# hannesweisbach/channelcoding

Hardware: AMD Instinct MI355X
Metric: decoded frames/sec (coded bits/sec = value x 255), BCH(255,231) min-sum, batch=2^20 (higher is better)
Workload: dtype f32

## Files before the change

channelcoding_amd/csrc/cc_internal.hpp:

```cpp
#pragma once
#include <hip/hip_runtime.h>

#include <cstdint>
#include <memory>
#include <mutex>
#include <string>
#include <vector>

#include "../../include/channelcoding_amd.h"
#include "galois.hpp"

namespace ccamd {

struct MinSumGeometry {
  int W = 64, C = 4, frames_per_wave = 1, KW = 1;
};

struct MinSumParams {
  int n, K, KW;
  int variant;
  int stop_rule;
  unsigned iterations;
  float alpha_f;
  float beta_f;
// ... 158 lines not shown
                           const uint32_t *d_er_off, uint8_t *d_out, int32_t *d_nerr, int32_t *d_status, size_t B,
                           hipStream_t stream, int il = 1);
int launch_chase(const cc_code *code, const float *d_llr, unsigned p, uint8_t *d_out, int32_t *d_nerr, float *d_metric,
                 int32_t *d_status, size_t B, hipStream_t stream);
int chase_frames_per_wave(const cc_code *code, unsigned p, bool soft, bool extended = false);
int launch_chase_soft(const cc_code *code, const float *d_llr, unsigned p, float beta, uint8_t *d_out, float *d_ext,
                      int32_t *d_nerr, float *d_metric, int32_t *d_status, size_t B, hipStream_t stream);
int launch_chase_extended(const cc_code *code, const float *d_llr, unsigned p, float beta, uint8_t *d_out, float *d_ext,
                          int32_t *d_nerr, float *d_metric, int32_t *d_status, size_t B, hipStream_t stream);
int launch_osd(const cc_code *code, const float *d_llr, unsigned order, uint8_t *d_out, int32_t *d_nerr, float *d_metric,
               int32_t *d_status, size_t B, hipStream_t stream);
int osd_frames_per_wave(const cc_code *code);
std::vector<unsigned long long> build_osd_rows(const CodeTables &t);
int launch_gmd(const cc_code *code, const uint8_t *d_words, const float *d_rel, unsigned m, uint8_t *d_out, int32_t *d_nerr,
               float *d_metric, int32_t *d_status, size_t B, hipStream_t stream);
bool bitslice_supported(const cc_code *code);
int launch_bitslice_syndromes(const cc_code *code, bool float_in, const void *d_in, uint8_t *d_out, uint8_t *d_synd, size_t B,
                              hipStream_t stream, int il = 1);
bool bitslice_encode_supported(const cc_code *code);
int launch_bitslice_encode(const cc_code *code, const uint8_t *d_msg, uint8_t *d_cw, size_t B, hipStream_t stream, int il = 1);
int launch_bitslice_chien(const void *d_lamp, void *d_masks, size_t B, bool long_locators, hipStream_t stream);
int launch_bitslice_roots_transpose(const void *d_masks, void *d_rootsT, size_t B, hipStream_t stream);
constexpr uint32_t kLogZero = 512;
int launch_chunk_bm(const cc_code *code, const uint8_t *d_synd, const uint16_t *d_er, const uint32_t *d_er_off,
                    uint16_t *d_llg, uint16_t *d_meta, unsigned long long *d_mask, uint8_t *d_lamp, int ncoef,
                    uint32_t *d_nleft, int32_t *d_nerr, int32_t *d_status, size_t B, hipStream_t stream);
int algebraic_route(const cc_code *code, size_t B, bool erasures);
bool planes_small_call(const cc_code *code, size_t B);
int launch_pgz_erasures(const cc_code *code, const uint8_t *d_in, const uint16_t *d_er, const uint32_t *d_er_off,
                        uint8_t *d_out, int32_t *d_nerr, int32_t *d_status, size_t B, hipStream_t stream);
constexpr int diag_variant_part(int variant, int parts) {
  const int order = variant == CC_ALG_MS ? 0 : variant == CC_ALG_NMS ? 1 : variant == CC_ALG_OMS ? 2
                  : variant == CC_ALG_SCMS2 ? 3 : variant == CC_ALG_SCMS1 ? 4 : 5;
  return order % parts;
}

enum DiagRowBody { DIAG_ROWS_BUTTERFLY = 0, DIAG_ROWS_FOUR = 1, DIAG_ROWS_FOUR_PIPELINED = 2, DIAG_ROWS_FOUR_ZIPPED = 3 };
constexpr int diag_row_body(int K, int D, int LPF, int variant) {
  const bool plain = variant == CC_ALG_MS || variant == CC_ALG_NMS || variant == CC_ALG_OMS || variant == CC_ALG_2DNMS;
  if (!(K == 24 && D == 7 && LPF == 16 && plain)) return DIAG_ROWS_BUTTERFLY;
#ifdef CC_DIAG_FOUR_ROW_BODY
  return CC_DIAG_FOUR_ROW_BODY;
#else
  return DIAG_ROWS_FOUR_ZIPPED;
#endif
}

constexpr bool diag_switch_from_registers(int K, int D, int LPF, int variant) {
  if (LPF != 8) return true;
  if (K == 28 && D == 7) return false;
  if (variant == CC_ALG_SCMS2) return !((K == 21 && D == 6) || (K == 10 && D == 1) || (K == 8 && D == 1));
  if (variant == CC_ALG_SCMS1) return !((K == 20 && D == 1) || (K == 24 && D == 4));
  return true;
}

int launch_wide_correct(const cc_code *code, const uint16_t *d_in, const uint16_t *d_er, const uint32_t *d_off,
                        uint16_t *d_out, int32_t *d_nerr, int32_t *d_status, size_t B, hipStream_t stream);
int launch_wide_pgz_erasures(const cc_code *code, const uint16_t *d_in, const uint16_t *d_er, const uint32_t *d_off,
                        uint16_t *d_out, int32_t *d_nerr, int32_t *d_status, size_t B, hipStream_t stream);
int launch_wide_encode(const cc_code *code, const uint16_t *d_msg, uint16_t *d_cw, size_t B, hipStream_t stream);
int launch_wide_extract(const cc_code *code, const uint16_t *d_cw, uint16_t *d_msg, size_t B, hipStream_t stream);
std::vector<uint8_t> build_parity_table(const Field &f, const CodeTables &t);
int launch_encode(const cc_code *code, const uint8_t *d_msg, uint8_t *d_cw, size_t B, hipStream_t stream);
int launch_encode_bits(const cc_code *code, const uint8_t *d_msg, uint8_t *d_cw, size_t B, hipStream_t stream);
int launch_extract(const cc_code *code, const uint8_t *d_cw, uint8_t *d_msg, size_t B, hipStream_t stream);
int launch_pack_bits(const void *d_sym, int width, size_t n, uint8_t *d_packed, size_t B, hipStream_t stream);
int launch_unpack_bits(const uint8_t *d_packed, size_t n, void *d_sym, int width, size_t B, hipStream_t stream);
bool packed_native_supported(const cc_code *code, size_t B);
int launch_packed_correct(const cc_code *code, const uint8_t *d_in, uint8_t *d_out, int32_t *d_nerr, int32_t *d_status,
                          size_t B, hipStream_t stream);
bool packed_long_supported(const cc_code *code, size_t B);
int launch_packed_long_correct(const cc_code *code, const uint8_t *d_in, uint8_t *d_out, int32_t *d_nerr, int32_t *d_status,
                               size_t B, hipStream_t stream);
bool packed_encode_native(const cc_code *code);
bool packed_extract_native(const cc_code *code);
int launch_packed_encode(const cc_code *code, const uint8_t *d_msg, uint8_t *d_cw, size_t B, hipStream_t stream);
int launch_packed_extract(const cc_code *code, const uint8_t *d_cw, uint8_t *d_msg, size_t B, hipStream_t stream);
constexpr size_t kInterleaveMax = 256;
constexpr size_t kInterleaveNativeMax = 16;
int launch_interleave(const void *d_in, int width, size_t n, size_t I, void *d_out, size_t B, bool to_interleaved,
                      hipStream_t stream);
bool interleaved_native_supported(const cc_code *code, size_t B, size_t I, bool erasures);
bool interleaved_encode_native(const cc_code *code, size_t I);
bool interleaved_extract_native(const cc_code *code, size_t I);
int launch_interleaved_extract(const cc_code *code, const void *d_cw, void *d_msg, size_t B, size_t I, hipStream_t stream);
struct ProductShape {
  int e;
  size_t w1, w2, k1, k2, N;
};
ProductShape product_shape(const cc_product *pc);
size_t product_chunk_blocks(size_t N, size_t blocks, size_t at_least = 1);
int launch_product_decode(const cc_product *pc, const float *d_y, uint8_t *d_out, float *d_ext, int32_t *d_status, size_t B,
                          hipStream_t stream);
int launch_product_encode(const cc_product *pc, const uint8_t *d_msg, uint8_t *d_cw, size_t B, hipStream_t stream);
int launch_product_extract(const cc_product *pc, const uint8_t *d_cw, uint8_t *d_msg, size_t B, hipStream_t stream);
int product_awgn(const cc_product *pc, double ebno_db, uint64_t seed, uint64_t first_block, size_t blocks,
                 int random_codewords, float *d_y, uint8_t *d_sent, hipStream_t stream);
int mc_run_product(const cc_product *pc, double ebno_db, uint64_t seed, uint64_t first_block, size_t blocks,
                   int random_codewords, uint64_t *d_counters, hipStream_t stream);
int mc_run_product_hard(const cc_product *pc, double ebno_db, uint64_t seed, uint64_t first_block, size_t blocks,
                        int random_codewords, uint64_t *d_counters, hipStream_t stream);
int launch_product_hard(const cc_product *pc, const uint8_t *d_in, uint8_t *d_out, int32_t *d_nflip, int32_t *d_last,
                        int32_t *d_status, size_t B, hipStream_t stream);
struct SrSchedule {
  int D = 0;
  float u[CC_PRODUCT_SR_MAX_LEVELS] = {};
// ... 74 lines not shown
```

channelcoding_amd/csrc/minsum_diag.hip:

```cpp
#include "minsum_diag_impl.hpp"

#include <algorithm>
#include <cstdlib>

namespace ccamd {

using DiagLaunch = int (*)(const cc_code *, const MinSumParams &, const float *, const uint16_t *, const uint32_t *,
                           uint8_t *, float *, uint16_t *, int32_t *, size_t, hipStream_t);
#define CC_PART_DECL(NAME, I)                                                                                        \
  int launch_minsum_diag_##NAME##_p##I(const cc_code *, const MinSumParams &, const float *, const uint16_t *,       \
                                       const uint32_t *, uint8_t *, float *, uint16_t *, int32_t *, size_t, hipStream_t);
#define CC_PARTS_1(M, NAME) M(NAME, 0)
#define CC_PARTS_2(M, NAME) CC_PARTS_1(M, NAME) M(NAME, 1)
#define CC_PARTS_3(M, NAME) CC_PARTS_2(M, NAME) M(NAME, 2)
#define CC_PARTS_6(M, NAME) CC_PARTS_3(M, NAME) M(NAME, 3) M(NAME, 4) M(NAME, 5)
#define GEO(NAME, N, KK, W, DD, LL, CC, OO, SC, PA, LK, PP) CC_PARTS_##PP(CC_PART_DECL, NAME)
#include "minsum_diag_geos.inc"
#undef GEO
namespace {
struct DiagEntry {
  DiagGeometry geo;
  int parts;
  DiagLaunch launch[6];
};
// ... 150 lines not shown
    return mx * 1000 + sq;
  };
  bool improved = true;
  while (improved) {
    improved = false;
    for (int a = 0; a < D && !improved; ++a)
      for (int b = a + 1; b < D && !improved; ++b)
        for (size_t x = 0; x < grp[a].size() && !improved; ++x)
          for (size_t y = 0; y < grp[b].size() && !improved; ++y) {
            const int before = group_cost(grp[a]) + group_cost(grp[b]);
            std::swap(grp[a][x], grp[b][y]);
            if (group_cost(grp[a]) + group_cost(grp[b]) < before)
              improved = true;
            else
              std::swap(grp[a][x], grp[b][y]);
          }
  }
  std::vector<uint16_t> out(static_cast<size_t>(D) * W, 0xFFFFu);
  for (int g = 0; g < D; ++g)
    for (size_t l = 0; l < grp[g].size(); ++l) out[g * W + l] = static_cast<uint16_t>(grp[g][l]);
  (void)real_last;
  return out;
}

bool minsum_diag_supported(const cc_code *code) {
  if (code->d_diag == nullptr || code->desc.iterations == 0) return false;
  const int alg = code->desc.algorithm;
  const DiagGeometry *geo = diag_geometry(code->tab);
  if (!geo) return false;
  if (alg == CC_ALG_SCMS1) return true;
  if (alg == CC_ALG_SCMS2) return geo->scms;
  if (alg != CC_ALG_MS && alg != CC_ALG_NMS && alg != CC_ALG_OMS && alg != CC_ALG_2DNMS) return false;
  if (alg == CC_ALG_OMS && !(code->desc.beta >= 0.0)) return false;
  const float a = static_cast<float>(code->desc.alpha);
  if ((alg == CC_ALG_NMS || alg == CC_ALG_2DNMS) && !(a == a && a - a == 0.0f)) return false;
  return diag_geometry(code->tab) != nullptr;
}


std::string minsum_diag_name(const cc_code *code) {
  const DiagGeometry *g = diag_geometry(code->tab);
  if (!g) return "minsum_diag_kernel";
  const int body = diag_row_body(static_cast<int>(g->k), g->D, g->LPF, code->desc.algorithm);
  return "minsum_diag_kernel<K=" + std::to_string(g->k) + ",D=" + std::to_string(g->D) + ",LPF=" + std::to_string(g->LPF) +
         (body == DIAG_ROWS_FOUR_ZIPPED      ? ",four-row-zipped>"
          : body == DIAG_ROWS_FOUR_PIPELINED ? ",four-row-pipelined>"
          : body == DIAG_ROWS_FOUR           ? ",four-row>"
                                             : ",row-pipelined>");
}

size_t minsum_diag_lds_bytes(const DiagGeometry &g) {
  const bool partial = g.w != static_cast<unsigned>(g.LPF * g.D);
  const size_t fpw = 64 / g.LPF, rc = static_cast<size_t>(g.LPF) * g.CPL + (partial ? 48 : (g.LPF == 8 && g.CPL == 8 ? 8 : 16));
  return 4 * (fpw * rc * 8 + (fpw / 2) * rc * 8) + 256 * 4 +
         4 * static_cast<size_t>(g.CPL) * 256;
}


namespace {

__global__ void __launch_bounds__(256)
twopass_gather_kernel(const uint32_t *__restrict__ ctl, unsigned sample, unsigned cap, const uint32_t *__restrict__ list,
                      const float *__restrict__ llr, float *__restrict__ llr2, int n) {
  if (!two_pass_in_effect(ctl, sample, cap)) return;
  const unsigned long long cnt = ctl[1];
  const int lane = threadIdx.x & 63;
  const unsigned long long nwaves = static_cast<unsigned long long>(gridDim.x) * 4;
  for (unsigned long long k = static_cast<unsigned long long>(blockIdx.x) * 4 + (threadIdx.x >> 6); k < cnt; k += nwaves) {
    const float *src = llr + static_cast<unsigned long long>(list[k]) * n;
    float *dst = llr2 + k * n;
    for (int j = lane; j < n; j += 64) dst[j] = src[j];
  }
}
__global__ void __launch_bounds__(256)
twopass_scatter_kernel(const uint32_t *__restrict__ ctl, unsigned sample, unsigned cap, const uint32_t *__restrict__ list,
                       const uint8_t *__restrict__ hard2, const uint16_t *__restrict__ iters2,
                       const int32_t *__restrict__ status2, uint8_t *__restrict__ hard, uint16_t *__restrict__ iters,
                       int32_t *__restrict__ status, int n) {
  if (!two_pass_in_effect(ctl, sample, cap)) return;
  const unsigned long long cnt = ctl[1];
  const int lane = threadIdx.x & 63;
  const unsigned long long nwaves = static_cast<unsigned long long>(gridDim.x) * 4;
  for (unsigned long long k = static_cast<unsigned long long>(blockIdx.x) * 4 + (threadIdx.x >> 6); k < cnt; k += nwaves) {
    const unsigned long long f = list[k];
    for (int j = lane; j < n; j += 64) hard[f * n + j] = hard2[k * n + j];
    if (lane == 0) {
      if (iters) iters[f] = iters2[k];
      if (status) status[f] = status2[k];
    }
  }
}

bool two_pass_enabled() { return minsum_shortcuts_enabled(); }

int launch_two_pass(const cc_code *code, const DiagEntry *e, const MinSumParams &p, const float *d_llr, uint8_t *d_hard,
                    uint16_t *d_iters, int32_t *d_status, size_t B, hipStream_t stream) {
  const size_t n = code->tab.n, cap = B / 4, sample = 4096;
  auto up = [](size_t v) { return (v + 255) & ~static_cast<size_t>(255); };
  constexpr size_t max_runs = 4, o_pool = 256, pool_bytes = POOL_WORDS * 4;
  const size_t o_list = o_pool + (max_runs + 2) * pool_bytes, o_llr = o_list + up(cap * 4), o_hard = o_llr + up(cap * n * 4),
               o_it = o_hard + up(cap * n), o_st = o_it + up(cap * 2), total = o_st + up(cap * 4);
  uint8_t *ws = nullptr;
  CC_HIP_TRY(workspace_alloc(code, reinterpret_cast<void **>(&ws), total, stream));
  uint32_t *ctl = reinterpret_cast<uint32_t *>(ws), *list = reinterpret_cast<uint32_t *>(ws + o_list);
  float *llr2 = reinterpret_cast<float *>(ws + o_llr);
  uint8_t *hard2 = ws + o_hard;
  uint16_t *it2 = reinterpret_cast<uint16_t *>(ws + o_it);
// ... 102 lines not shown
```

channelcoding_amd/csrc/minsum_diag_impl.hpp:

```cpp
#pragma once
#include <cstdio>
#include <cstdlib>
#include <type_traits>
#include <utility>

#include "cc_internal.hpp"
#include "wave_ops.hpp"


namespace ccamd {
namespace {



template <int... Is, typename F>
__device__ __forceinline__ void static_for_impl(std::integer_sequence<int, Is...>, F &&f) {
  (f(std::integral_constant<int, Is>{}), ...);
}
template <int N, typename F>
__device__ __forceinline__ void static_for(F &&f) {
  static_for_impl(std::make_integer_sequence<int, N>{}, static_cast<F &&>(f));
}
template <int... Gs>
struct PairGaps {
// ... 170 lines not shown
__device__ __forceinline__ int signum(float v) { return (0.0f < v) - (v < 0.0f); }
template <int VARIANT>
__device__ __forceinline__ float self_correct(float tmp, float q_old) {
  if constexpr (VARIANT == CC_ALG_SCMS1) {
    const int so = signum(q_old);
    return (so == 0 || so == signum(tmp)) ? tmp : 0.0f;
  } else {
    return (tmp * q_old > 0.0f) ? tmp : 0.5f * (tmp + q_old);
  }
}

template <int VARIANT>
__device__ __forceinline__ float horizontal(float m, float alpha_f, double beta_d) {
  if constexpr (VARIANT == CC_ALG_NMS || VARIANT == CC_ALG_2DNMS) {
    return __fmul_rn(alpha_f, m);
  } else if constexpr (VARIANT == CC_ALG_OMS) {
    const double a = static_cast<double>(m) - beta_d;
    return static_cast<float>((a < 0.0) ? 0.0 : a);
  } else {
    return m;
  }
}

template <int K, int D, int VARIANT, int RB, int LPF, int CPL, int OCC, bool PARTIAL, typename PG = PairGaps<>,
          bool SINGLE = false, bool CHAIN = false, int BODY = DIAG_ROWS_BUTTERFLY>
__global__ void __launch_bounds__(256, OCC)
minsum_diag_kernel(MinSumParams p, const uint16_t *__restrict__ diag_s, const uint32_t *__restrict__ colbits,
                   const float *__restrict__ llr, const uint16_t *__restrict__ er, const uint32_t *__restrict__ er_off,
                   uint8_t *__restrict__ hard, float *__restrict__ Lout, uint16_t *__restrict__ iters_out,
                   int32_t *__restrict__ status_out, unsigned long long B) {
  static_assert(K % RB == 0 && K <= 32, "row batching");
  if (p.gate == 1 && !two_pass_sampled(p)) return;
  if (p.dual && two_pass_in_effect(p.ctl, p.sample, p.list_cap)) {
    llr = p.llr2;
    hard = p.hard2;
    Lout = nullptr;
    iters_out = p.iters2;
    status_out = p.status2;
    B = p.ctl[1] < p.list_cap ? p.ctl[1] : p.list_cap;
  }
  static_assert(LPF == 8 || LPF == 16, "a frame occupies half or all of a 16-lane DPP row");
  static_assert(2 * PG::NP <= D && !(PARTIAL && PG::NP > 0), "paired slots");
  static_assert(!CHAIN || PG::NP == 0 || (PG::gap(0) == 1 && PG::gap(PG::NP - 1) == 1), "links are gap-1 pairs");
  constexpr int NLK = CHAIN ? PG::NP : 0;
  constexpr int FPW = 64 / LPF;
  constexpr int RC = LPF * CPL + (PARTIAL ? 48 : (LPF == 8 && CPL == 8 ? 8 : 16));
  extern __shared__ __attribute__((aligned(16))) char smem[];
  constexpr int CY_BYTES = FPW * RC * 8, CN_BYTES = (FPW / 2) * RC * 8;
  constexpr int WAVE_BYTES = CY_BYTES + (SINGLE ? 0 : CN_BYTES);
  const int lane = threadIdx.x & 63, wid = threadIdx.x >> 6;
  const int fl = lane / LPF, lam = lane & (LPF - 1);
  char *cy_base = smem + wid * WAVE_BYTES;
  char *cn_lane = cy_base + CY_BYTES + ((fl >> 1) - fl) * RC * 8 + (fl & 1) * 4;
  uint32_t *cbits = reinterpret_cast<uint32_t *>(smem + 4 * WAVE_BYTES);
  char *stg = smem + 4 * WAVE_BYTES + 1024 + wid * (CPL * 256);
  const uint32_t stg_lds = __builtin_amdgcn_readfirstlane(static_cast<uint32_t>(reinterpret_cast<size_t>(stg)));
  cbits[threadIdx.x] = colbits[threadIdx.x];
  constexpr bool POOL = !SINGLE && LPF == 16;
  __shared__ unsigned wg_next;
  if (!POOL && threadIdx.x == 0) wg_next = 2 * 4 * (64 / LPF);
  __syncthreads();

  const int n = p.n;
  int aCY[D];
#pragma unroll
  for (int d = 0; d < D; ++d) aCY[d] = (fl * RC + diag_s[d * LPF + lam]) * 8;
  float pen = 0.0f;
  uint32_t sgn_keep = 0xFFFFFFFFu;
  if constexpr (PARTIAL) {
    if (diag_s[(D - 1) * LPF + lam] == 0xFFFFu) {
      aCY[D - 1] = (fl * RC + LPF * CPL + 16) * 8;
      pen = 3.402823466e+38f;
      sgn_keep = 0u;
    }
  }
  const int col0 = fl * RC + lam;
  const bool oddf = SINGLE && (fl & 1);
#ifndef CC_EXP_O0_B32
  auto cell_y = [&](float2 v) -> float { return SINGLE ? (oddf ? v.x : v.y) : v.y; };
  auto cell_cs = [&](float2 v) -> float { return SINGLE ? (oddf ? v.y : v.x) : v.x; };
#else
  auto cell_y = [&](float2 v) -> float { return v.y; };
  auto cell_cs = [&](float2 v) -> float { return v.x; };
#endif
  auto make_cell = [&](float cs, float y) -> float2 { return (SINGLE && oddf) ? make_float2(y, cs) : make_float2(cs, y); };
  const int y_off = (SINGLE && oddf) ? 0 : 4;
  int aWR[SINGLE ? D : 1];
  if constexpr (SINGLE) {
#pragma unroll
    for (int d = 0; d < D; ++d) aWR[d] = aCY[d] + (oddf ? 4 : 0);
  }

  constexpr unsigned GPW = 4 * FPW;
  const unsigned S = gridDim.x < POOL_SHARDS ? gridDim.x : POOL_SHARDS, shard = blockIdx.x % S, Ws = (gridDim.x - shard + S - 1) / S;
  const unsigned obase = 2 * Ws * GPW;
  auto frame_of = [&](unsigned o) -> unsigned long long { return static_cast<unsigned long long>(o) * S + shard; };
  auto draw = [&]() -> unsigned {
    uint32_t line = shard * 32;
    asm volatile("" : "+v"(line));
    return atomicAdd(p.pool + line, 1u);
  };
  auto drawn = [&](unsigned o) -> unsigned {
    return obase + static_cast<unsigned>(__builtin_amdgcn_ds_bpermute((lane & ~(LPF - 1)) * 4, static_cast<int>(o)));
  };
  __shared__ uint2 ords[POOL ? GPW : 1];
  uint2 &my_ords = ords[POOL ? wid * FPW + fl : 0];
  unsigned opd = 0;
  constexpr bool PREDRAW = !(VARIANT == CC_ALG_SCMS1 && K * D < 160);
  const unsigned long long ngroups = static_cast<unsigned long long>(gridDim.x) * GPW;
  auto ordinal_frame = [&](unsigned o) -> unsigned long long {
    return static_cast<unsigned long long>(blockIdx.x) * GPW + (o % GPW) + static_cast<unsigned long long>(o / GPW) * ngroups;
  };
  auto take_frame = [&]() -> unsigned long long {
    unsigned o = 0;
    if (lam == 0) o = atomicAdd(&wg_next, 1u);
    o = static_cast<unsigned>(__builtin_amdgcn_ds_bpermute((lane & ~(LPF - 1)) * 4, static_cast<int>(o)));
    return ordinal_frame(o);
  };
  unsigned long long frame, nextf;
  if constexpr (POOL) {
    const unsigned ofr = (blockIdx.x / S) * GPW + wid * FPW + fl;
    if (lam == 0) my_ords = make_uint2(ofr, ofr + Ws * GPW);
    frame = frame_of(ofr);
    nextf = frame_of(ofr + Ws * GPW);
  } else {
    frame = (static_cast<unsigned long long>(blockIdx.x) * 4 + wid) * FPW + fl;
    nextf = frame + ngroups;
  }
  bool active = frame < B;
  unsigned it = 0;
  constexpr bool NEEDQ = (VARIANT == CC_ALG_SCMS1 || VARIANT == CC_ALG_SCMS2);
  constexpr bool QONLY = !SINGLE && ((VARIANT == CC_ALG_SCMS2 && 2 * K * D + 64 > 256) ||
                                     (VARIANT == CC_ALG_SCMS1 && K * D >= 160 && OCC >= 2));
  constexpr bool KEEPQ = (VARIANT == CC_ALG_SCMS2 && !SINGLE) || QONLY;
  float R[(SINGLE || QONLY) ? 1 : K][(SINGLE || QONLY) ? 1 : D];
  float Q[KEEPQ ? K : 1][KEEPQ ? D : 1];
  __shared__ uint2 row_state[QONLY ? 4 * FPW * K : 1];
  uint2 *const my_rows = row_state + (QONLY ? (wid * FPW + fl) * K : 0);
  uint2 rsq = make_uint2(0u, 0u);
  constexpr bool BITS1 = VARIANT == CC_ALG_SCMS1 && !SINGLE && !QONLY;
  constexpr int RPW = 32 / D;
  constexpr int NW = (K + RPW - 1) / RPW;
  uint32_t SW[BITS1 ? NW : 1], ZW[BITS1 ? NW : 1];

  constexpr bool X4 = (LPF * CPL - 1) >= 4 * LPF;
  constexpr int NF = (LPF * CPL - 1) / (4 * LPF);
  auto stage = [&](unsigned long long f) {
    if (f < B) {
      const float *src = llr + f * n;
      if constexpr (X4) {
        const float *v = src + 4 * lam;
        const float *vt = v + (n - 4 * LPF);
        uint32_t m0_save;
        const uint32_t sb = __builtin_amdgcn_readfirstlane(stg_lds);
        static_assert(NF == 1 || NF == 3, "x4 staging is written out for one or three aligned copies");
        if constexpr (NF == 3) {
          asm volatile(
              "s_mov_b32 %0, m0\n\ts_mov_b32 m0, %3\n\ts_nop 0\n\tglobal_load_lds_dwordx4 %1, off\n\t"
              "s_add_u32 m0, %3, %4\n\ts_nop 0\n\tglobal_load_lds_dwordx4 %1, off offset:%7\n\t"
              "s_add_u32 m0, %3, %5\n\ts_nop 0\n\tglobal_load_lds_dwordx4 %1, off offset:%8\n\t"
              "s_add_u32 m0, %3, %6\n\ts_nop 0\n\tglobal_load_lds_dwordx4 %2, off\n\ts_mov_b32 m0, %0"
              : "=&s"(m0_save)
              : "v"(v), "v"(vt), "s"(sb), "n"(1024 - LPF * 16), "n"(2048 - 2 * LPF * 16), "n"(3072), "n"(LPF * 16),
                "n"(2 * LPF * 16)
              : "memory", "scc");
        } else {
          asm volatile(
              "s_mov_b32 %0, m0\n\ts_mov_b32 m0, %3\n\ts_nop 0\n\tglobal_load_lds_dwordx4 %1, off\n\t"
              "s_add_u32 m0, %3, 1024\n\ts_nop 0\n\tglobal_load_lds_dwordx4 %2, off\n\ts_mov_b32 m0, %0"
              : "=&s"(m0_save)
              : "v"(v), "v"(vt), "s"(sb)
              : "memory", "scc");
        }
      } else {
#pragma unroll
        for (int c = 0; c < CPL; ++c) {
          const int j = lam + LPF * c;
          if (j < n) {
            uint32_t m0_save;
            asm volatile("s_mov_b32 %0, m0\n\ts_mov_b32 m0, %2\n\ts_nop 0\n\tglobal_load_lds_dword %1, off\n\ts_mov_b32 m0, %0"
                         : "=&s"(m0_save) : "v"(src + j), "s"(stg_lds + c * 256) : "memory");
          }
        }
      }
    }
  };
  const char *stg_full = stg + fl * LPF * 16 + lam * 4;
  const char *stg_tail = stg + NF * 1024 + fl * LPF * 16 + (lam - n + 4 * LPF) * 4;
  auto staged = [&](int c) -> float {
    if constexpr (X4) {
      if (c < 4 * NF) return *reinterpret_cast<const float *>(stg_full + (c / 4) * 1024 + (c % 4) * 4 * LPF);
      return *reinterpret_cast<const float *>(stg_tail + 4 * LPF * c);
    } else {
      return *reinterpret_cast<const float *>(stg + c * 256 + lane * 4);
    }
  };
  auto setup = [&](unsigned long long f) {
#pragma unroll
    for (int c = 0; c < CPL; ++c) {
      float y = staged(c) + 0.0f;
      if (c == CPL - 1 && lam + LPF * c >= n) y = 0.0f;
      *reinterpret_cast<float2 *>(cy_base + (col0 + LPF * c) * 8) = make_cell(0.0f, y);
    }
    if (er_off != nullptr) {
      for (uint32_t e = er_off[f]; e < er_off[f + 1]; ++e) {
        const int pos = er[e];
        if ((pos & (LPF - 1)) == lam) *reinterpret_cast<float *>(cy_base + (fl * RC + pos) * 8 + y_off) = 0.0f;
      }
    }
    if constexpr (!SINGLE && !QONLY) static_for<K>([&](auto I) { static_for<D>([&](auto Dd) { R[I][Dd] = 0.0f; }); });
    if constexpr (KEEPQ) static_for<K>([&](auto I) { static_for<D>([&](auto Dd) { Q[I][Dd] = 0.0f; }); });
    if constexpr (QONLY)
      for (int r = lam; r < K; r += LPF) my_rows[r] = make_uint2(0u, 0u);
    if constexpr (BITS1) static_for<NW>([&](auto Wd) { SW[Wd] = 0u; ZW[Wd] = 0xFFFFFFFFu; });
  };

#pragma unroll
  for (int c = 0; c < CPL; ++c)
    if constexpr (!SINGLE) *reinterpret_cast<float *>(cn_lane + (col0 + LPF * c) * 8) = 0.0f;
  if (active) {
    stage(frame);
    asm volatile("s_waitcnt vmcnt(0)" ::: "memory");
    setup(frame);
    stage(nextf);
    if (POOL && PREDRAW && lam == 0) opd = draw();
  }

  while (__any(active)) {
    constexpr bool PREFETCH = !(BITS1 && K * D >= 160) && !SINGLE;
    constexpr bool TRED = BODY != DIAG_ROWS_BUTTERFLY;
    static_assert(!TRED || (LPF == 16 && K % 4 == 0 && !SINGLE && !NEEDQ),
                  "four rows per reduction: a frame per DPP row, whole row groups, plain variants (the self-correcting ones spill)");
    constexpr bool READY = TRED && VARIANT == CC_ALG_MS;
    constexpr bool EARLY_PF = TRED && PREFETCH;
    float2 cyq[D];
    float2 carry_cy[NLK ? NLK : 1];
    float carry_sum[NLK ? NLK : 1];
    auto fetch = [&](auto IC) {
      constexpr int row = decltype(IC)::value;
      if constexpr (QONLY) rsq = my_rows[row];
      static_for<D>([&](auto DD) {
        constexpr int d = TRED ? D - 1 - DD : DD;
        if constexpr (d < 2 * NLK && (d & 1) == 0 && row >= 1) {
// ... 16 lines not shown
      });
    };
    float Tloc[D];
    auto row_front = [&](auto IR, uint32_t &o1, uint32_t &o2, uint32_t &os, auto &&mid) {
      constexpr int i = decltype(IR)::value;
      if constexpr (!PREFETCH) fetch(IR);
      [[maybe_unused]] auto wget = [&](auto DD) -> float {
        if constexpr (SINGLE) return Tloc[DD];
        else if constexpr (QONLY) return Q[i][DD];
        else return R[i][DD];
      };
      auto wset = [&](auto DD, float v) {
        if constexpr (SINGLE) Tloc[DD] = v;
        else if constexpr (!QONLY) R[i][DD] = v;
      };
      [[maybe_unused]] const float old_hi = u2f(rsq.y & 0x7FFFFFFFu);
      [[maybe_unused]] uint32_t old_Y = (rsq.x ^ rsq.y);
      if constexpr (QONLY) asm volatile("" : "+v"(old_Y));
      {
        float a1 = 0.0f, a2 = (D == 1) ? 3.402823466e+38f : 0.0f;
        uint32_t s = 0;
        uint32_t qs[D];
        float mag[D], qv[D];
        uint32_t keep = 0;
        constexpr int wi = BITS1 ? i / RPW : 0, sh = BITS1 ? (i % RPW) * D : 0;
        if constexpr (BITS1) {
          uint32_t tw = 0, tz = 0;
          static_for<D>([&](auto DD) {
            constexpr int d = DD;
            const float t = (cyq[d].x - R[i][d]) + cyq[d].y;
            R[i][d] = t;
            tw = __builtin_amdgcn_alignbit(tw, f2u(t), 31);
            tz = shift_in_is_zero(tz, t);
          });
          constexpr uint32_t field = ((D == 32 ? 0u : (1u << D)) - 1u) << sh;
          const uint32_t tws = tw << sh, tzs = tz << sh;
          keep = ZW[wi] | ~(SW[wi] ^ tws);
          SW[wi] = (SW[wi] & ~field) | (tws & keep);
          ZW[wi] = (ZW[wi] & ~field) | ((~keep & field) | tzs);
        }
        static_for<D>([&](auto DD) {
          constexpr int d = DD;
          float q;
          if constexpr (BITS1) {
            const int32_t m = __builtin_amdgcn_sbfe(static_cast<int32_t>(keep), sh + D - 1 - d, 1);
            q = u2f(f2u(R[i][d]) & static_cast<uint32_t>(m));
          } else if constexpr (SINGLE) {
            q = cell_y(cyq[d]);
            if constexpr (NEEDQ) q = self_correct<VARIANT>(q, 0.0f);
          } else {
            float r_old;
            if constexpr (QONLY) r_old = u2f(f2u(__builtin_amdgcn_fmed3f(Q[i][d], -old_hi, old_hi)) ^ old_Y);
            else r_old = R[i][d];
            float e = cyq[d].x - r_old;
            if constexpr (VARIANT == CC_ALG_2DNMS) e = __fmul_rn(p.beta_f, e);
            q = e + cyq[d].y;
            if constexpr (QONLY && VARIANT == CC_ALG_SCMS1) {
              const uint32_t so = f2u(Q[i][d]), st = f2u(q);
              const int differ = static_cast<int>(so ^ st) >> 31;
              const uint32_t zero_old = umin32(so, 1u) - 1u;
              q = u2f(static_cast<uint32_t>(__builtin_amdgcn_bitop3_b32(static_cast<int>(st), static_cast<int>(zero_old), differ,
                                                                        0xD0)));
              Q[i][d] = q;
            } else if constexpr (KEEPQ) {
              q = self_correct<VARIANT>(q, Q[i][d]);
              Q[i][d] = q;
            }
          }
          wset(DD, q);
          qv[d] = q;
        });
        if constexpr (EARLY_PF) {
          static_for<NLK>([&](auto P) { carry_cy[P] = cyq[2 * P + 1]; });
          asm volatile("" ::: "memory");
          if constexpr (i + 1 < K) fetch(std::integral_constant<int, i + 1>{});
          asm volatile("" ::: "memory");
        }
        mid();
        static_for<D>([&](auto DD) {
          constexpr int d = DD;
          const float q = qv[d];
          float a = __builtin_fabsf(q);
          uint32_t qb = f2u(q);
          if constexpr (PARTIAL && d == D - 1) {
            a = __builtin_fmaxf(a, pen);
            qb &= sgn_keep;
          }
          qs[d] = qb;
          constexpr bool RAW = (SINGLE || BITS1) && !PARTIAL && D >= 2;
          mag[d] = RAW ? q : a;
          if constexpr (D == 2 && d == 1) {
            a2 = RAW ? max_abs2(mag[0], mag[1]) : __builtin_fmaxf(mag[0], mag[1]);
            a1 = RAW ? min_abs2(mag[0], mag[1]) : __builtin_fminf(mag[0], mag[1]);
          } else if constexpr (d == 0 && D == 1) {
            a1 = a;
          } else if constexpr (d == 2) {
            a2 = RAW ? med3_abs3(mag[0], mag[1], mag[2]) : __builtin_amdgcn_fmed3f(mag[0], mag[1], mag[2]);
            a1 = RAW ? min3_abs3(mag[0], mag[1], mag[2]) : __builtin_fminf(__builtin_fminf(mag[0], mag[1]), mag[2]);
          } else if constexpr (d >= 4 && (d & 1) == 0) {
            const float md = RAW ? med3_abs23(a1, mag[d - 1], mag[d]) : __builtin_amdgcn_fmed3f(a1, mag[d - 1], mag[d]);
            a1 = RAW ? min3_abs23(a1, mag[d - 1], mag[d]) : __builtin_fminf(__builtin_fminf(a1, mag[d - 1]), mag[d]);
            a2 = __builtin_fminf(a2, md);
          } else if constexpr (d == D - 1 && d >= 3 && (d & 1) == 1) {
            a2 = RAW ? med3_abs1(a1, mag[d], a2) : __builtin_amdgcn_fmed3f(a1, mag[d], a2);
            a1 = RAW ? min_abs1(a1, mag[d]) : __builtin_fminf(a1, mag[d]);
          }
        });
// ... 118 lines not shown
          if constexpr (!READY) b2 = bank_bcast<J>(ZC[g]);
          row_back(std::integral_constant<int, 4 * g + J>{}, b0, b1, b2, cn);
        });
      };
      auto alone = [](auto) {};
      if constexpr (BODY == DIAG_ROWS_FOUR_ZIPPED) {
        float cn[D];
        auto back_step = [&](auto IG, auto J) {
          constexpr int i = 4 * decltype(IG)::value + decltype(J)::value;
          __builtin_amdgcn_sched_barrier(0);
          const uint32_t b0 = bank_bcast<J>(ZA[IG]), b1 = bank_bcast<J>(ZB[IG]);
          uint32_t b2 = 0;
          if constexpr (!READY) b2 = bank_bcast<J>(ZC[IG]);
          row_back(std::integral_constant<int, i>{}, b0, b1, b2, cn);
          if constexpr (i + 1 < K) row_cn(std::integral_constant<int, i + 1>{}, cn);
          asm volatile("" ::: "memory");
          __builtin_amdgcn_sched_barrier(0);
        };
        fronts(std::integral_constant<int, 0>{}, alone);
        row_cn(std::integral_constant<int, 0>{}, cn);
        asm volatile("" ::: "memory");
        static_for<NG - 1>([&](auto IG) {
          fronts(std::integral_constant<int, IG + 1>{}, [&](auto J) { back_step(IG, J); });
        });
        static_for<4>([&](auto J) { back_step(std::integral_constant<int, NG - 1>{}, J); });
      } else if constexpr (BODY == DIAG_ROWS_FOUR_PIPELINED) {
        fronts(std::integral_constant<int, 0>{}, alone);
        static_for<NG>([&](auto IG) {
          if constexpr (IG + 1 < NG) fronts(std::integral_constant<int, IG + 1>{}, alone);
          backs(IG);
        });
      } else {
        static_for<NG>([&](auto IG) {
          fronts(IG, alone);
          backs(IG);
        });
      }
    } else {
      static_for<K>([&](auto IR) {
        uint32_t m1[1], m2[1], sg[1];
        row_front(IR, m1[0], m2[0], sg[0], [] {});
        float cn[D];
        row_cn(IR, cn);
#ifndef CC_EXP_NO_REDUCE
        row_allreduce<1, LPF>(m1, m2, sg);
#endif
        row_back(IR, m1[0], m2[0], sg[0], cn);
      });
    }

    uint32_t acc = 0;
    constexpr bool REGSW = SINGLE || diag_switch_from_registers(K, D, LPF, VARIANT);
    float cnv[CPL], yc[CPL];
    auto stop_scan = [&](auto ORC) {
      uint32_t cb[CPL];
#pragma unroll
      for (int c = 0; c < CPL; ++c) {
        if constexpr (SINGLE) {
          const float2 cy = *reinterpret_cast<const float2 *>(cy_base + (col0 + LPF * c) * 8);
          cnv[c] = cy.x;
          yc[c] = cy.y;
        } else {
          cnv[c] = *reinterpret_cast<const float *>(cn_lane + (col0 + LPF * c) * 8);
          yc[c] = *reinterpret_cast<const float *>(cy_base + (col0 + LPF * c) * 8 + 4);
        }
        cb[c] = cbits[lam + LPF * c];
      }
      asm volatile("" ::: "memory");
#pragma unroll
      for (int c = 0; c < CPL; ++c) {
        const int m = static_cast<int>(f2u(cnv[c] + yc[c])) >> 31;
        if constexpr (decltype(ORC)::value)
          acc = static_cast<uint32_t>(__builtin_amdgcn_bitop3_b32(static_cast<int>(acc), m, static_cast<int>(cb[c]), 0xF8));
        else
          acc = static_cast<uint32_t>(__builtin_amdgcn_bitop3_b32(static_cast<int>(acc), m, static_cast<int>(cb[c]), 0x78));
      }
      if constexpr (!SINGLE) {
#pragma unroll
        for (int c = 0; c < CPL; ++c) {
          *reinterpret_cast<float *>(cy_base + (col0 + LPF * c) * 8) = cnv[c];
          *reinterpret_cast<float *>(cn_lane + (col0 + LPF * c) * 8) = 0.0f;
        }
      }
    };
    bool ok;
    if (SINGLE && p.stop_rule == CC_STOP_AS_SHIPPED) {
      ok = true;
#pragma unroll
      for (int c = 0; c < CPL; ++c) {
        const float2 cy = *reinterpret_cast<const float2 *>(cy_base + (col0 + LPF * c) * 8);
        cnv[c] = cy.x;
        yc[c] = cy.y;
      }
      asm volatile("" ::: "memory");
    } else if (p.stop_rule == CC_STOP_PUBLISHED) {
      stop_scan(std::true_type{});
      ok = group_or<LPF>(acc) == 0;
    } else {
      stop_scan(std::false_type{});
      ok = (p.stop_rule == CC_STOP_AS_SHIPPED) || group_xor<LPF>(acc) == 0;
    }
#ifdef CC_EXP_NEVER_STOP
    ok = false;
#endif
    const bool finished = SINGLE || ok || (it + 1 >= p.iterations);
    if (finished && active) {
      const uint2 od = POOL ? my_ords : make_uint2(0u, 0u);
      const unsigned long long done = POOL ? frame_of(od.x) : frame;
      const unsigned done_it = ok ? it : p.iterations;
      frame = POOL ? frame_of(od.y) : nextf;
      active = frame < B;
      uint8_t *hp = hard + done * n + lam;
      float *Lp = Lout ? Lout + done * n + lam : nullptr;
      bool handed = false;
      if constexpr (SINGLE) handed = p.first_pass != 0 && !ok;
      auto emit_col = [&](int c, float L, bool want_L) {
        if (c < CPL - 1 || lam + LPF * c < n) {
          hp[LPF * c] = (L < 0.0f) ? 1 : 0;
          if (want_L) Lp[LPF * c] = L;
        }
      };
      auto emit = [&](auto WANT_L) {
#pragma unroll
        for (int c = 0; c < CPL; ++c) emit_col(c, cnv[c] + yc[c], decltype(WANT_L)::value);
      };
      auto emit_frame = [&] {
        if (handed) return;
        if (Lout) emit(std::true_type{});
        else emit(std::false_type{});
      };
      if (active) {
        if constexpr (!REGSW) {
          asm volatile("s_waitcnt vmcnt(0)" ::: "memory");
#pragma unroll
          for (int c = 0; c < CPL; ++c) {
            const float2 cy = *reinterpret_cast<const float2 *>(cy_base + (col0 + LPF * c) * 8);
            float y = staged(c) + 0.0f;
            if (c == CPL - 1 && lam + LPF * c >= n) y = 0.0f;
            *reinterpret_cast<float2 *>(cy_base + (col0 + LPF * c) * 8) = make_cell(0.0f, y);
            emit_col(c, cy.x + cy.y, Lp != nullptr);
          }
        } else {
          asm volatile("s_waitcnt vmcnt(0)" ::: "memory");
          if constexpr (SINGLE) emit_frame();
          float ys[CPL];
#pragma unroll
          for (int c = 0; c < CPL; ++c) ys[c] = staged(c);
          asm volatile("" ::: "memory");
          if constexpr (!SINGLE) emit_frame();
#pragma unroll
          for (int c = CPL - 1; c >= 0; --c) {
            float y = ys[c] + 0.0f;
            if (c == CPL - 1 && lam + LPF * c >= n) y = 0.0f;
            *reinterpret_cast<float2 *>(cy_base + (col0 + LPF * c) * 8) = make_cell(0.0f, y);
          }
        }
        if (er_off != nullptr) {
          for (uint32_t e = er_off[frame]; e < er_off[frame + 1]; ++e) {
            const int pos = er[e];
            if ((pos & (LPF - 1)) == lam) *reinterpret_cast<float *>(cy_base + (fl * RC + pos) * 8 + y_off) = 0.0f;
          }
        }
        if constexpr (!SINGLE && !QONLY) static_for<K>([&](auto I) { static_for<D>([&](auto Dd) { R[I][Dd] = 0.0f; }); });
        if constexpr (KEEPQ) static_for<K>([&](auto I) { static_for<D>([&](auto Dd) { Q[I][Dd] = 0.0f; }); });
        if constexpr (QONLY)
          for (int r = lam; r < K; r += LPF) my_rows[r] = make_uint2(0u, 0u);
        if constexpr (BITS1) static_for<NW>([&](auto Wd) { SW[Wd] = 0u; ZW[Wd] = 0xFFFFFFFFu; });
        it = 0;
      } else if constexpr (REGSW) {
        emit_frame();
      } else {
#pragma unroll
        for (int c = 0; c < CPL; ++c) {
          const float2 cy = *reinterpret_cast<const float2 *>(cy_base + (col0 + LPF * c) * 8);
          emit_col(c, cy.x + cy.y, Lp != nullptr);
        }
      }
      if (lam == 0) {
        if (handed) {
          if (p.first_pass == 2) {
            atomicAdd(&p.ctl[2], 1u);
          } else {
            const uint32_t at = atomicAdd(&p.ctl[1], 1u);
            if (at < p.list_cap) p.list[at] = static_cast<uint32_t>(done);
            else p.ctl[3] = 1u;
          }
        } else {
          if (iters_out) iters_out[done] = static_cast<uint16_t>(done_it);
          if (status_out) status_out[done] = ok ? CC_FRAME_OK : CC_FRAME_NOT_CONVERGED;
        }
      }
      if (active) {
        if constexpr (POOL) {
          if (!PREDRAW && lam == 0) opd = draw();
          const unsigned nx = drawn(opd);
          stage(frame_of(nx));
          if (lam == 0) {
            my_ords = make_uint2(od.y, nx);
            if (PREDRAW) opd = draw();
          }
        } else {
          nextf = take_frame();
          stage(nextf);
        }
      }
    } else {
      ++it;
    }
  }
  asm volatile("s_waitcnt vmcnt(0)" ::: "memory");
}

}

namespace {

template <int K, int D, int LPF, int CPL, int OCC, bool SCMS = false, bool PARTIAL = false, typename PG = PairGaps<>,
          bool CHAIN = false, int PARTS = 1, int PART = 0>
int launch_diag_geometry(const cc_code *code, const MinSumParams &p, const float *d_llr, const uint16_t *d_er,
                         const uint32_t *d_er_off, uint8_t *d_hard, float *d_L, uint16_t *d_iters, int32_t *d_status,
                         size_t B, hipStream_t stream) {
  constexpr int RB = 1;
  constexpr bool Q_ONLY_2 = 2 * K * D + 64 > 256, Q_ONLY_1 = K * D >= 160 && OCC >= 2;
  constexpr int OCC_S = Q_ONLY_2 ? OCC : (2 * K * D + 64 <= 128) ? 4 : (2 * K * D + 64 <= 168) ? 3 : 2;
  constexpr int FPW = 64 / LPF;
  if (!(code->tab.n > static_cast<unsigned>(LPF * (CPL - 1)) && code->tab.n <= static_cast<unsigned>(LPF * CPL))) {
    set_last_error("minsum_diag: only the last owned column of a lane may lie beyond the frame");
    return CC_ERR_UNSUPPORTED;
  }
  if (p.pool == nullptr || B >= (1ull << 32)) {
    set_last_error("minsum_diag: no frame pool, or more than 2^32 frames in one call");
    return CC_ERR_UNSUPPORTED;
  }
  const DiagGeometry g{0, 0, PARTIAL ? 1u : static_cast<unsigned>(LPF * D), D, LPF, CPL, SCMS};
  const size_t lds = minsum_diag_lds_bytes(g);
  const unsigned long long blocks_needed = (B + 4 * FPW - 1) / (4 * FPW);
  constexpr size_t ords_bytes = LPF == 16 ? 4 * FPW * sizeof(uint2) : 0;
  unsigned long long per_cu = (160 * 1024) / (lds + ords_bytes);
  const unsigned long long occ = p.variant == CC_ALG_SCMS2 ? static_cast<unsigned long long>(OCC_S) : OCC;
  if ((p.variant == CC_ALG_SCMS2 && Q_ONLY_2) || (p.variant == CC_ALG_SCMS1 && Q_ONLY_1))
    per_cu = (160 * 1024) / (lds + ords_bytes + 4 * FPW * K * sizeof(uint2));
  if (per_cu > occ) per_cu = occ;
  const unsigned long long max_grid = static_cast<unsigned long long>(code->num_cus) * per_cu;
  const int grid = static_cast<int>(blocks_needed < max_grid ? blocks_needed : max_grid);
  const unsigned long long Bq = B;
  hipError_t e = hipSuccess;
  const bool single = p.stop_rule == CC_STOP_AS_SHIPPED || p.iterations == 1 || p.first_pass != 0;
  constexpr size_t rc_cols = static_cast<size_t>(LPF) * CPL + (PARTIAL ? 48 : (LPF == 8 && CPL == 8 ? 8 : 16));
  const size_t lds_s = lds - 4 * (FPW / 2) * rc_cols * 8;
  unsigned long long per_cu_s = (160 * 1024) / lds_s;
  if (per_cu_s > 8) per_cu_s = 8;
  const unsigned long long max_grid_s = static_cast<unsigned long long>(code->num_cus) * per_cu_s;
  const int grid_s = static_cast<int>(blocks_needed < max_grid_s ? blocks_needed : max_grid_s);
#define CC_LAUNCH_S(V, O, S)                                                                                       \
  {                                                                                                                \
    const size_t lds_k = (S) ? lds_s : lds;                                                                        \
    const int grid_k = (S) ? grid_s : grid;                                                                        \
    e = hipFuncSetAttribute(                                                                                       \
        reinterpret_cast<const void *>(&minsum_diag_kernel<K, D, V, RB, LPF, CPL, O, PARTIAL, PG, S, CHAIN,        \
                                                           (S) ? DIAG_ROWS_BUTTERFLY : diag_row_body(K, D, LPF, V)>), \
        hipFuncAttributeMaxDynamicSharedMemorySize, static_cast<int>(lds_k));                                     \
    if (e == hipSuccess)                                                                                           \
      hipLaunchKernelGGL((minsum_diag_kernel<K, D, V, RB, LPF, CPL, O, PARTIAL, PG, S, CHAIN,                        \
                                             (S) ? DIAG_ROWS_BUTTERFLY : diag_row_body(K, D, LPF, V)>),               \
                         dim3(grid_k), dim3(256), lds_k, stream, p, code->d_diag, code->d_colbits, d_llr, d_er,    \
                         d_er_off, d_hard, d_L, d_iters,                                                           \
                         d_status, Bq);                                                                            \
  }
#define CC_LAUNCH(V, O)                                                                                            \
  {                                                                                                                \
    if constexpr (diag_variant_part(V, PARTS) != PART) e = hipErrorInvalidValue;                                   \
    else if (single) CC_LAUNCH_S(V, OCC, true) else CC_LAUNCH_S(V, O, false)                                       \
  }
  switch (p.variant) {
    case CC_ALG_MS: CC_LAUNCH(CC_ALG_MS, OCC) break;
    case CC_ALG_NMS: CC_LAUNCH(CC_ALG_NMS, OCC) break;
    case CC_ALG_OMS: CC_LAUNCH(CC_ALG_OMS, OCC) break;
    case CC_ALG_2DNMS: CC_LAUNCH(CC_ALG_2DNMS, OCC) break;
    case CC_ALG_SCMS1:
      CC_LAUNCH(CC_ALG_SCMS1, OCC)
      break;
    case CC_ALG_SCMS2:
      if constexpr (SCMS) CC_LAUNCH(CC_ALG_SCMS2, OCC_S) else e = hipErrorInvalidValue;
      break;
    default: e = hipErrorInvalidValue;
  }
#undef CC_LAUNCH
#undef CC_LAUNCH_S
  if (e == hipSuccess) e = hipGetLastError();
  if (e != hipSuccess) return hip_fail(e, "minsum_diag kernel launch");
// ... 7 lines not shown
```

Measured before the change: 73.32 million.

## Skip per-frame message reset via stale-start scaling, wide CN zeroing, lane-major masks

For the BCH(255,231) plain min-sum geometry, frame switches no longer zero the per-row R registers. A scale factor g (0 on the first iteration of a new frame, -1 afterwards) folds the old message into the subtraction, and R is cleared only when a non-finite value shows up. Per-frame iteration counts come from a wave iteration counter minus a stamp kept in LDS. The CN area is zeroed with wide 16-byte stores across the whole wave instead of per-lane scalar stores, and column masks are stored lane-major so each lane reads them with uint4 loads. This removes register and LDS clearing work on frame turnover, at the cost of an extra FMA per message, more LDS for ords and masks, and subtle correctness conditions.

```diff
diff --git a/channelcoding_amd/csrc/cc_internal.hpp b/channelcoding_amd/csrc/cc_internal.hpp
--- a/channelcoding_amd/csrc/cc_internal.hpp
+++ b/channelcoding_amd/csrc/cc_internal.hpp
@@ -234,6 +234,23 @@
   if (variant == CC_ALG_SCMS2) return !((K == 21 && D == 6) || (K == 10 && D == 1) || (K == 8 && D == 1));
   if (variant == CC_ALG_SCMS1) return !((K == 20 && D == 1) || (K == 24 && D == 4));
   return true;
+}
+
+#ifndef CC_DIAG_NO_E49
+#define CC_DIAG_NO_E49 0
+#endif
+constexpr bool diag_masks_by_lane(int LPF, int CPL) { return LPF == 16 && CPL == 16 && !(CC_DIAG_NO_E49 & 4); }
+constexpr int diag_mask_table_bytes(int LPF, int CPL) { return diag_masks_by_lane(LPF, CPL) ? 16 * 80 : 256 * 4; }
+constexpr bool diag_zero_wave_wide(int K, int D, int LPF, int variant) {
+  const bool plain = variant == CC_ALG_MS || variant == CC_ALG_NMS || variant == CC_ALG_OMS || variant == CC_ALG_2DNMS;
+  if (LPF != 16 || (CC_DIAG_NO_E49 & 2)) return false;
+  return K == 24 && D == 7 && plain;
+}
+constexpr bool diag_start_on_stale_messages(int K, int D, int LPF, int variant, bool partial) {
+  const bool plain = variant == CC_ALG_MS || variant == CC_ALG_NMS || variant == CC_ALG_OMS || variant == CC_ALG_2DNMS;
+  if (LPF != 16 || partial || !plain || (CC_DIAG_NO_E49 & 1)) return false;
+  if (!(K == 24 && D == 7)) return false;
+  return diag_switch_from_registers(K, D, LPF, variant);
 }
 
 int launch_wide_correct(const cc_code *code, const uint16_t *d_in, const uint16_t *d_er, const uint32_t *d_off,
diff --git a/channelcoding_amd/csrc/minsum_diag.hip b/channelcoding_amd/csrc/minsum_diag.hip
--- a/channelcoding_amd/csrc/minsum_diag.hip
+++ b/channelcoding_amd/csrc/minsum_diag.hip
@@ -226,7 +226,7 @@
 size_t minsum_diag_lds_bytes(const DiagGeometry &g) {
   const bool partial = g.w != static_cast<unsigned>(g.LPF * g.D);
   const size_t fpw = 64 / g.LPF, rc = static_cast<size_t>(g.LPF) * g.CPL + (partial ? 48 : (g.LPF == 8 && g.CPL == 8 ? 8 : 16));
-  return 4 * (fpw * rc * 8 + (fpw / 2) * rc * 8) + 256 * 4 +
+  return 4 * (fpw * rc * 8 + (fpw / 2) * rc * 8) + static_cast<size_t>(diag_mask_table_bytes(g.LPF, g.CPL)) +
          4 * static_cast<size_t>(g.CPL) * 256;
 }
 
diff --git a/channelcoding_amd/csrc/minsum_diag_impl.hpp b/channelcoding_amd/csrc/minsum_diag_impl.hpp
--- a/channelcoding_amd/csrc/minsum_diag_impl.hpp
+++ b/channelcoding_amd/csrc/minsum_diag_impl.hpp
@@ -246,10 +246,15 @@
   const int fl = lane / LPF, lam = lane & (LPF - 1);
   char *cy_base = smem + wid * WAVE_BYTES;
   char *cn_lane = cy_base + CY_BYTES + ((fl >> 1) - fl) * RC * 8 + (fl & 1) * 4;
+  constexpr bool MASKS_BY_LANE = diag_masks_by_lane(LPF, CPL);
+  constexpr int MASK_BYTES = diag_mask_table_bytes(LPF, CPL);
   uint32_t *cbits = reinterpret_cast<uint32_t *>(smem + 4 * WAVE_BYTES);
-  char *stg = smem + 4 * WAVE_BYTES + 1024 + wid * (CPL * 256);
+  char *stg = smem + 4 * WAVE_BYTES + MASK_BYTES + wid * (CPL * 256);
+  constexpr bool ZERO_WIDE = !SINGLE && diag_zero_wave_wide(K, D, LPF, VARIANT);
+  [[maybe_unused]] const uint32_t cn_area_off = __builtin_amdgcn_readfirstlane(static_cast<uint32_t>(wid * WAVE_BYTES + CY_BYTES));
   const uint32_t stg_lds = __builtin_amdgcn_readfirstlane(static_cast<uint32_t>(reinterpret_cast<size_t>(stg)));
-  cbits[threadIdx.x] = colbits[threadIdx.x];
+  if constexpr (MASKS_BY_LANE) cbits[(threadIdx.x & (LPF - 1)) * 20 + threadIdx.x / LPF] = colbits[threadIdx.x];
+  else cbits[threadIdx.x] = colbits[threadIdx.x];
   constexpr bool POOL = !SINGLE && LPF == 16;
   __shared__ unsigned wg_next;
   if (!POOL && threadIdx.x == 0) wg_next = 2 * 4 * (64 / LPF);
@@ -297,8 +302,11 @@
   auto drawn = [&](unsigned o) -> unsigned {
     return obase + static_cast<unsigned>(__builtin_amdgcn_ds_bpermute((lane & ~(LPF - 1)) * 4, static_cast<int>(o)));
   };
-  __shared__ uint2 ords[POOL ? GPW : 1];
-  uint2 &my_ords = ords[POOL ? wid * FPW + fl : 0];
+  constexpr bool STALE = !SINGLE && POOL && diag_start_on_stale_messages(K, D, LPF, VARIANT, PARTIAL);
+  constexpr int OW = STALE ? 4 : 2;
+  __shared__ __attribute__((aligned(16))) unsigned ords[POOL ? GPW * OW : 2];
+  uint2 &my_ords = *reinterpret_cast<uint2 *>(&ords[POOL ? (wid * FPW + fl) * OW : 0]);
+  unsigned &my_stamp = ords[POOL ? (wid * FPW + fl) * OW + (STALE ? 2 : 0) : 0];
   unsigned opd = 0;
   constexpr bool PREDRAW = !(VARIANT == CC_ALG_SCMS1 && K * D < 160);
   const unsigned long long ngroups = static_cast<unsigned long long>(gridDim.x) * GPW;
@@ -323,6 +331,11 @@
   }
   bool active = frame < B;
   unsigned it = 0;
+  [[maybe_unused]] float g = 0.0f;
+  [[maybe_unused]] unsigned wit = 0;
+  if constexpr (STALE) {
+    if (lam == 0) my_stamp = 0u;
+  }
   constexpr bool NEEDQ = (VARIANT == CC_ALG_SCMS1 || VARIANT == CC_ALG_SCMS2);
   constexpr bool QONLY = !SINGLE && ((VARIANT == CC_ALG_SCMS2 && 2 * K * D + 64 > 256) ||
                                      (VARIANT == CC_ALG_SCMS1 && K * D >= 160 && OCC >= 2));
@@ -338,12 +351,13 @@
   uint32_t SW[BITS1 ? NW : 1], ZW[BITS1 ? NW : 1];
 
   constexpr bool X4 = (LPF * CPL - 1) >= 4 * LPF;
+  [[maybe_unused]] int sw_lam = lam, sw_fl = fl;
   constexpr int NF = (LPF * CPL - 1) / (4 * LPF);
   auto stage = [&](unsigned long long f) {
     if (f < B) {
       const float *src = llr + f * n;
       if constexpr (X4) {
-        const float *v = src + 4 * lam;
+        const float *v = src + 4 * (STALE ? sw_lam : lam);
         const float *vt = v + (n - 4 * LPF);
         uint32_t m0_save;
         const uint32_t sb = __builtin_amdgcn_readfirstlane(stg_lds);
@@ -382,7 +396,12 @@
   const char *stg_full = stg + fl * LPF * 16 + lam * 4;
   const char *stg_tail = stg + NF * 1024 + fl * LPF * 16 + (lam - n + 4 * LPF) * 4;
   auto staged = [&](int c) -> float {
-    if constexpr (X4) {
+    if constexpr (X4 && STALE) {
+      const char *sw_full = stg + sw_fl * LPF * 16 + sw_lam * 4;
+      const char *sw_tail = stg + NF * 1024 + sw_fl * LPF * 16 + (sw_lam - n + 4 * LPF) * 4;
+      if (c < 4 * NF) return *reinterpret_cast<const float *>(sw_full + (c / 4) * 1024 + (c % 4) * 4 * LPF);
+      return *reinterpret_cast<const float *>(sw_tail + 4 * LPF * c);
+    } else if constexpr (X4) {
       if (c < 4 * NF) return *reinterpret_cast<const float *>(stg_full + (c / 4) * 1024 + (c % 4) * 4 * LPF);
       return *reinterpret_cast<const float *>(stg_tail + 4 * LPF * c);
     } else {
@@ -505,7 +524,9 @@
             float r_old;
             if constexpr (QONLY) r_old = u2f(f2u(__builtin_amdgcn_fmed3f(Q[i][d], -old_hi, old_hi)) ^ old_Y);
             else r_old = R[i][d];
-            float e = cyq[d].x - r_old;
+            float e;
+            if constexpr (STALE) e = __builtin_fmaf(r_old, g, cyq[d].x);
+            else e = cyq[d].x - r_old;
             if constexpr (VARIANT == CC_ALG_2DNMS) e = __fmul_rn(p.beta_f, e);
             q = e + cyq[d].y;
             if constexpr (QONLY && VARIANT == CC_ALG_SCMS1) {
@@ -730,8 +751,21 @@
     uint32_t acc = 0;
     constexpr bool REGSW = SINGLE || diag_switch_from_registers(K, D, LPF, VARIANT);
     float cnv[CPL], yc[CPL];
+    [[maybe_unused]] unsigned stamp = 0;
     auto stop_scan = [&](auto ORC) {
       uint32_t cb[CPL];
+      if constexpr (STALE) stamp = my_stamp;
+      if constexpr (MASKS_BY_LANE) {
+        const uint4 *mine = reinterpret_cast<const uint4 *>(cbits + lam * 20);
+#pragma unroll
+        for (int c = 0; c < CPL; c += 4) {
+          const uint4 v = mine[c / 4];
+          cb[c] = v.x;
+          cb[c + 1] = v.y;
+          cb[c + 2] = v.z;
+          cb[c + 3] = v.w;
+        }
+      }
 #pragma unroll
       for (int c = 0; c < CPL; ++c) {
         if constexpr (SINGLE) {
@@ -742,7 +776,7 @@
           cnv[c] = *reinterpret_cast<const float *>(cn_lane + (col0 + LPF * c) * 8);
           yc[c] = *reinterpret_cast<const float *>(cy_base + (col0 + LPF * c) * 8 + 4);
         }
-        cb[c] = cbits[lam + LPF * c];
+        if constexpr (!MASKS_BY_LANE) cb[c] = cbits[lam + LPF * c];
       }
       asm volatile("" ::: "memory");
 #pragma unroll
@@ -757,7 +791,19 @@
 #pragma unroll
         for (int c = 0; c < CPL; ++c) {
           *reinterpret_cast<float *>(cy_base + (col0 + LPF * c) * 8) = cnv[c];
-          *reinterpret_cast<float *>(cn_lane + (col0 + LPF * c) * 8) = 0.0f;
+          if constexpr (!ZERO_WIDE) *reinterpret_cast<float *>(cn_lane + (col0 + LPF * c) * 8) = 0.0f;
+        }
+        if constexpr (ZERO_WIDE) {
+          static_assert(CN_BYTES % 16 == 0 && CY_BYTES % 16 == 0 && WAVE_BYTES % 16 == 0 && CN_BYTES >= 1024, "CN area in 16-byte stores");
+          uint32_t zl;
+          asm volatile("v_mbcnt_lo_u32_b32 %0, -1, 0\n\tv_mbcnt_hi_u32_b32 %0, -1, %0" : "=v"(zl));
+          char *cn_area = smem + cn_area_off;
+          constexpr int FULL = CN_BYTES / 1024, REST = CN_BYTES % 1024;
+#pragma unroll
+          for (int k = 0; k < FULL; ++k) *reinterpret_cast<float4 *>(cn_area + 1024 * k + 16 * zl) = make_float4(0.0f, 0.0f, 0.0f, 0.0f);
+          if constexpr (REST == 256) *reinterpret_cast<float *>(cn_area + 1024 * FULL + 4 * zl) = 0.0f;
+          else if constexpr (REST == 512) *reinterpret_cast<float2 *>(cn_area + 1024 * FULL + 8 * zl) = make_float2(0.0f, 0.0f);
+          else if constexpr (REST != 0) *reinterpret_cast<float4 *>(cn_area + CN_BYTES - 1024 + 16 * zl) = make_float4(0.0f, 0.0f, 0.0f, 0.0f);
         }
       }
     };
@@ -781,15 +827,22 @@
 #ifdef CC_EXP_NEVER_STOP
     ok = false;
 #endif
+    if constexpr (STALE) it = wit - stamp;
     const bool finished = SINGLE || ok || (it + 1 >= p.iterations);
     if (finished && active) {
+      if constexpr (STALE) {
+        uint32_t ln;
+        asm volatile("v_mbcnt_lo_u32_b32 %0, -1, 0\n\tv_mbcnt_hi_u32_b32 %0, -1, %0" : "=v"(ln));
+        sw_lam = static_cast<int>(ln & (LPF - 1));
+        sw_fl = static_cast<int>(ln / LPF);
+      }
       const uint2 od = POOL ? my_ords : make_uint2(0u, 0u);
       const unsigned long long done = POOL ? frame_of(od.x) : frame;
       const unsigned done_it = ok ? it : p.iterations;
       frame = POOL ? frame_of(od.y) : nextf;
       active = frame < B;
-      uint8_t *hp = hard + done * n + lam;
-      float *Lp = Lout ? Lout + done * n + lam : nullptr;
+      uint8_t *hp = hard + done * n + (STALE ? sw_lam : lam);
+      float *Lp = Lout ? Lout + done * n + (STALE ? sw_lam : lam) : nullptr;
       bool handed = false;
       if constexpr (SINGLE) handed = p.first_pass != 0 && !ok;
       auto emit_col = [&](int c, float L, bool want_L) {
@@ -839,11 +892,25 @@
             if ((pos & (LPF - 1)) == lam) *reinterpret_cast<float *>(cy_base + (fl * RC + pos) * 8 + y_off) = 0.0f;
           }
         }
-        if constexpr (!SINGLE && !QONLY) static_for<K>([&](auto I) { static_for<D>([&](auto Dd) { R[I][Dd] = 0.0f; }); });
-        if constexpr (KEEPQ) static_for<K>([&](auto I) { static_for<D>([&](auto Dd) { Q[I][Dd] = 0.0f; }); });
-        if constexpr (QONLY)
-          for (int r = lam; r < K; r += LPF) my_rows[r] = make_uint2(0u, 0u);
-        if constexpr (BITS1) static_for<NW>([&](auto Wd) { SW[Wd] = 0u; ZW[Wd] = 0xFFFFFFFFu; });
+        if constexpr (STALE) {
+          uint32_t um = 0u;
+          int32_t im = 0;
+#pragma unroll
+          for (int c = 0; c < CPL; ++c) {
+            um = umax32(um, f2u(cnv[c]));
+            im = static_cast<int32_t>(f2u(cnv[c])) > im ? static_cast<int32_t>(f2u(cnv[c])) : im;
+          }
+          const uint32_t big = umax32(um & 0x7FFFFFFFu, static_cast<uint32_t>(im));
+          if (group_or<LPF>(big >= 0x7F800000u ? 1u : 0u) != 0u)
+            static_for<K>([&](auto I) { static_for<D>([&](auto Dd) { R[I][Dd] = 0.0f; }); });
+          g = 0.0f;
+        } else {
+          if constexpr (!SINGLE && !QONLY) static_for<K>([&](auto I) { static_for<D>([&](auto Dd) { R[I][Dd] = 0.0f; }); });
+          if constexpr (KEEPQ) static_for<K>([&](auto I) { static_for<D>([&](auto Dd) { Q[I][Dd] = 0.0f; }); });
+          if constexpr (QONLY)
+            for (int r = lam; r < K; r += LPF) my_rows[r] = make_uint2(0u, 0u);
+          if constexpr (BITS1) static_for<NW>([&](auto Wd) { SW[Wd] = 0u; ZW[Wd] = 0xFFFFFFFFu; });
+        }
         it = 0;
       } else if constexpr (REGSW) {
         emit_frame();
@@ -875,6 +942,7 @@
           stage(frame_of(nx));
           if (lam == 0) {
             my_ords = make_uint2(od.y, nx);
+            if constexpr (STALE) my_stamp = wit + 1;
             if (PREDRAW) opd = draw();
           }
         } else {
@@ -884,7 +952,9 @@
       }
     } else {
       ++it;
+      if constexpr (STALE) g = -1.0f;
     }
+    if constexpr (STALE) wit = __builtin_amdgcn_readfirstlane(wit + 1);
   }
   asm volatile("s_waitcnt vmcnt(0)" ::: "memory");
 }
@@ -913,7 +983,7 @@
   const DiagGeometry g{0, 0, PARTIAL ? 1u : static_cast<unsigned>(LPF * D), D, LPF, CPL, SCMS};
   const size_t lds = minsum_diag_lds_bytes(g);
   const unsigned long long blocks_needed = (B + 4 * FPW - 1) / (4 * FPW);
-  constexpr size_t ords_bytes = LPF == 16 ? 4 * FPW * sizeof(uint2) : 0;
+  constexpr size_t ords_bytes = LPF == 16 ? 4 * FPW * sizeof(uint4) : 0;
   unsigned long long per_cu = (160 * 1024) / (lds + ords_bytes);
   const unsigned long long occ = p.variant == CC_ALG_SCMS2 ? static_cast<unsigned long long>(OCC_S) : OCC;
   if ((p.variant == CC_ALG_SCMS2 && Q_ONLY_2) || (p.variant == CC_ALG_SCMS1 && Q_ONLY_1))
```

Result: no change. 73.75 million (median of 6 runs) (+0.6%).
